# tiiuae/MLAdversarialObjectDetection

Hardware: AMD Instinct MI355X
Metric: patch-opt images/sec (EffDet-D0 512px fwd+bwd) (higher is better)
Workload: dtype f32; 1 GPU; C2: EfficientDet-D0 patch attack 512x512, 16 images/GPU, bn=local; global_batch=16, image_size=512, placement=injected, parallelism=dp1

## Files before the change

mladversarialobjectdetection_amd/csrc/api.cpp:

```cpp
#include "ctx.hpp"

namespace {

std::string json_escape(const std::string& s) {
  std::string o;
  for (char c : s) {
    if (c == '"' || c == '\\') o.push_back('\\');
    o.push_back(c);
  }
  return o;
}

std::vector<float> make_anchors(const ModelConfig& mc) {
  std::vector<int> fs{mc.image_size};
  int f = mc.image_size;
  for (int l = 1; l <= mc.max_level; ++l) {
    f = (f - 1) / 2 + 1;
    fs.push_back(f);
  }
  std::vector<float> out;
  for (int level = mc.min_level; level <= mc.max_level; ++level) {
    const double stride = (double)fs[0] / (double)fs[level];
    struct C { double base_x, base_y, ax, ay; };
    std::vector<C> cs;
// ... 589 lines not shown
  run_nms(ctx, E, 1, E.nms2_boxes, E.nms2_scores, E.nms2_count, s);
  launch_count_ge(E.nms2_scores, E.nms2_count, B, PHX_MAX_OUT, 0.5f, metrics + PHX_M_ASR_NUM, s);
  launch_tv(params, PHX_PATCH_SIZE, E.tvs, metrics, add_tv != 0, s);
  if (out_boxes) PHX_HIP(hipMemcpyAsync(out_boxes, E.nms2_boxes, (size_t)B * PHX_MAX_OUT * 16, hipMemcpyDeviceToDevice, s));
  if (out_scores) PHX_HIP(hipMemcpyAsync(out_scores, E.nms2_scores, (size_t)B * PHX_MAX_OUT * 4, hipMemcpyDeviceToDevice, s));
  if (out_count) PHX_HIP(hipMemcpyAsync(out_count, E.nms2_count, (size_t)B * 4, hipMemcpyDeviceToDevice, s));
  return PHX_OK;
  PHX_CATCH(ctx)
}

int phx_profile(phx_ctx* ctx, int enable) {
  if (!ctx) return PHX_EINVAL;
  ctx->prof.on = enable != 0;
  ctx->prof.recs.clear();
  ctx->prof.used = 0;
  return PHX_OK;
}

int phx_profile_report(phx_ctx* ctx, char* buf, size_t cap, size_t* needed) {
  if (!ctx) return PHX_EINVAL;
  PHX_TRY(ctx)
  if (buf && cap && !ctx->prof.report.empty()) {
    const std::string out = std::move(ctx->prof.report);
    ctx->prof.report.clear();
    if (needed) *needed = out.size() + 1;
    const size_t c = std::min(cap - 1, out.size());
    memcpy(buf, out.data(), c);
    buf[c] = 0;
    return PHX_OK;
  }
// ... 179 lines not shown
```

mladversarialobjectdetection_amd/csrc/ctx.hpp:

```cpp
#pragma once
#include <hip/hip_runtime.h>

#include <algorithm>
#include <array>
#include <cmath>
#include <cstdlib>
#include <cstring>
#include <exception>
#include <map>
#include <memory>
#include <sstream>
#include <string>
#include <functional>
#include <vector>

#include "common.hpp"
#include "env.hpp"
#include "exec_plan.hpp"
#include "kernels.hpp"
#include "model.hpp"
#include "phx.h"
#include "post.hpp"
#include "unet.hpp"

// ... 284 lines not shown
  size_t idx;
  hipStream_t s;
  std::string dbg;
  ExtTiming ext;
  Scope(phx_ctx* ctx, const char* kind, double flops, double bytes, hipStream_t st, const std::string& tag = "")
      : p(ctx->prof.on ? &ctx->prof : nullptr), s(st) {
    if (debug_sync()) {
      dbg = std::string(kind) + tag;
      PHX_HIP(hipStreamSynchronize(s));
    }
    if (!p) return;
    const double peak = (ctx->bf16 && std::string(kind) == "gemm") ? 2500.0 : 157.3;
    Prof::Rec r{std::string(kind) + (prof_detail() ? tag : std::string()), p->ev(), p->ev(), flops, bytes, peak};
    PHX_HIP(hipEventRecord(r.a, s));
    p->recs.push_back(r);
    idx = p->recs.size() - 1;
    if (std::string(kind) == "gemm") {
      ext = ExtTiming{r.a, r.b, false};
      ext_timing() = &ext;
    }
  }
  ~Scope() noexcept(false) {
    if (p) {
      if (ext_timing() == &ext) ext_timing() = nullptr;
      if (!ext.used) (void)hipEventRecord(p->recs[idx].b, s);
    }
    if (!dbg.empty() && std::uncaught_exceptions() == 0) {
      const hipError_t e = hipStreamSynchronize(s);
      if (e != hipSuccess) throw HipError(std::string("device error after ") + dbg + ": " + hipGetErrorString(e));
    }
// ... 34 lines not shown
```

mladversarialobjectdetection_amd/csrc/exec.cpp:

```cpp
#include "ctx.hpp"

constexpr size_t kMaxExecs = 4;

namespace {

void alloc_exec(Exec& E, int A) {
  const Program& P = E.prog;
  const int B = E.B;
  E.act = E.alloc<float>(E.abf ? (P.act_floats + 1) / 2 : P.act_floats);
  E.grad = E.alloc<float>(E.tag != 0 ? 1 : P.grad_floats);
  E.slot_a.assign(P.n_slots, nullptr);
  E.slot_b.assign(P.n_slots, nullptr);
  E.slot_c.assign(P.n_slots, nullptr);
  E.slot_d.assign(P.n_slots, nullptr);
  E.slot_e.assign(P.n_slots, nullptr);
  for (const Op& op : P.ops) {
    const Tensor& ti = P.tensors[op.in[0]];
    if (op.t == OP_BN) {
      E.slot_a[op.slot] = E.alloc<float>(ti.c);
      E.slot_b[op.slot] = E.alloc<float>(ti.c);
      E.slot_c[op.slot] = E.alloc<float>(ti.c);
      E.slot_d[op.slot] = E.alloc<float>(ti.c);
      E.slot_e[op.slot] = E.alloc<float>(ti.c);
      PHX_HIP(hipMemset(E.slot_d[op.slot], 0, ti.c * sizeof(float)));
// ... 957 lines not shown

}

phx::ExtTiming*& phx::ext_timing() {
  static ExtTiming* t = nullptr;
  return t;
}

phx::ProfScope phx::prof_begin(phx_ctx* ctx, const char* kind, double flops, double bytes, hipStream_t s) {
  ProfScope r{nullptr, 0, s};
  if (!ctx || !ctx->prof.on) return r;
  Prof* p = &ctx->prof;
  Prof::Rec rec{kind, p->ev(), p->ev(), flops, bytes, 157.3};
  PHX_HIP(hipEventRecord(rec.a, s));
  p->recs.push_back(rec);
  r.p = p;
  r.idx = p->recs.size() - 1;
  return r;
}

void phx::prof_end(const ProfScope& r) {
  if (r.p) PHX_HIP(hipEventRecord(static_cast<Prof*>(r.p)->recs[r.idx].b, r.s));
}
```

mladversarialobjectdetection_amd/csrc/kernels.hpp:

```cpp
#pragma once
#include <hip/hip_runtime.h>
#include <hip/hip_ext.h>

#include <cstddef>
#include <cstdint>

#include "common.hpp"

namespace phx {

struct ExtTiming {
  hipEvent_t a = nullptr, b = nullptr;
  bool used = false;
};
ExtTiming*& ext_timing();
#define PHX_TLAUNCH(K, G, BL, SHM, S, ...)                                                              \
  do {                                                                                                 \
    if (::phx::ExtTiming* t_ = ::phx::ext_timing()) {                                                  \
      hipExtLaunchKernelGGL(K, G, BL, SHM, S, t_->used ? nullptr : t_->a, t_->b, 0, __VA_ARGS__);      \
      t_->used = true;                                                                                 \
    } else {                                                                                           \
      hipLaunchKernelGGL(K, G, BL, SHM, S, __VA_ARGS__);                                               \
    }                                                                                                  \
  } while (0)
// ... 101 lines not shown
};
bool sep_bwd_supported(int C, int N, bool bf16);
void launch_sep_bwd(const SepBwdMember* m, int n, int B, int C, int N, const float* wd, const float* wp,
                    hipStream_t s, int* nps);
void launch_dw_fwd_fused(const FuseView& fv, const float* w, float* y, int B, int H, int W, int C, int Ho,
                         int Wo, int k, int stride, int pt, int pl, hipStream_t s);
void launch_dw_bwd_group(const DwSeg* segs, int n, int B, int C, const float* w, int k, int stride,
                         hipStream_t s, int* nps);
struct DwTileInfo {
  int lcg, rpt, otw, oth, nrg, rin, cin, tiles_x, ntiles, ncg;
  int small;
  long wgs;
};
DwTileInfo dw_tile_info(int H, int W, int C, int Ho, int Wo, int pt, int pl, int k, int stride, bool bwd);
DwTileInfo dw_fused_tile_info(int B, int H, int W, int C, int Ho, int Wo, int pt, int pl);
struct SepTileInfo {
  int tw, th, tiles_x, ntiles;
};
SepTileInfo sep_tile_info(int H, int W);
struct StemPlanInfo {
  int blocks, last_valid, tiles_x, tiles_y, last_qx, last_qy;
};
StemPlanInfo stem_plan_info(int B, int H, int W);
struct Conv3PlanInfo {
  int G, xr, sweeps;
  long tiles, tper;
  int xcd_tiles[8], xcd_wgs[8];
};
Conv3PlanInfo conv3_small_plan_info(long M);

// ... 161 lines not shown
```

mladversarialobjectdetection_amd/csrc/kernels_dw.hip:

```cpp
#include <algorithm>
#include <cstdlib>
#include <stdexcept>
#include <type_traits>

#include "env.hpp"
#include "dw_stage.hpp"
#include "kernels.hpp"

namespace phx {

struct DwGeom {
  int H, W, C;
  int Ho, Wo;
  int pt, pl;
  int lcg;
  int otw, oth;
  int nrg;
  int rin, cin;
  int tiles_x, ntiles, ncg;
  int per;
};

template <class XV>
struct DwFwdSegT {
  XV x;
  float* y;
  DwGeom g;
  StatSink sink;
};
using DwFwdSeg = DwFwdSegT<InX>;
template <int NS, class XV = InX>
struct DwFwdGroup {
  DwFwdSegT<XV> s[NS];
  const float* w;
};
// ... 75 lines not shown
}

template <class Src, int U = 4>
__device__ __forceinline__ void dw_stage(float4* tile, const Src& src, int b, int sh, int sw, int C,
                                         int r0, int c0, int chan, const DwGeom& g) {
  if constexpr (Src::kActT) {
    const int act = src.act();
    if (act == 1) dw_stage_t<1, Src, U>(tile, src, b, sh, sw, C, r0, c0, chan, g);
    else if (act == 2) dw_stage_t<2, Src, U>(tile, src, b, sh, sw, C, r0, c0, chan, g);
    else dw_stage_t<0, Src, U>(tile, src, b, sh, sw, C, r0, c0, chan, g);
  } else {
    dw_stage_t<0, Src, U>(tile, src, b, sh, sw, C, r0, c0, chan, g);
  }
}

__device__ __forceinline__ float4 dw_xor_sum(float4 v, int lcg) {
  for (int o = 1 << lcg; o < 64; o <<= 1) {
    v.x += __shfl_xor(v.x, o);
    v.y += __shfl_xor(v.y, o);
    v.z += __shfl_xor(v.z, o);
    v.w += __shfl_xor(v.w, o);
  }
  return v;
}

template <int RPT>
__device__ __forceinline__ void dw_stats(const float4 (&acc)[RPT], unsigned vmask, int lcg, int c,
                                         long p, const StatSink& sink) {
  __shared__ float4 wm_[4][8], w2_[4][8];
  __shared__ float wn_[4][8];
// ... 27 lines not shown
#pragma unroll
    for (int w = 0; w < 4; ++w) {
      const float4 a = wm_[w][cg], b = w2_[w][cg];
      const float nn = wn_[w][cg];
      chan_merge(tn[0], tm[0], t2[0], nn, a.x, b.x);
      chan_merge(tn[1], tm[1], t2[1], nn, a.y, b.y);
      chan_merge(tn[2], tm[2], t2[2], nn, a.z, b.z);
      chan_merge(tn[3], tm[3], t2[3], nn, a.w, b.w);
    }
#pragma unroll
    for (int j = 0; j < 4; ++j) sink_put(sink, p, c + j, tn[j], tm[j], t2[j]);
    if (threadIdx.x == 0) sink_cnt(sink, p, tn[0]);
  }
}

template <int K, int S, int RPT, bool STATS, int NS, class XV, int SU = 4, bool BF = false>
__global__ __launch_bounds__(256) void k_dw_fwd(DwFwdGroup<NS, XV> grp) {
  using Stage = std::conditional_t<std::is_same<XV, InX>::value, StageInX<BF>, StageFuse<BF>>;
  const DwFwdSegT<XV> sg = pick_seg(grp.s, NS == 1 ? 0 : (int)blockIdx.y);
  const XV& xv = sg.x;
  const DwGeom& g = sg.g;
  const StatSink& sink = sg.sink;
  const float* __restrict__ w = grp.w;
  float* __restrict__ y = sg.y;
  extern __shared__ float4 tile[];
  const int b = blockIdx.z;
  int tl, cgi;
  if (!dw_block_map(blockIdx.x, g.per, g.ncg, g.ntiles * g.ncg, &tl, &cgi)) return;
  const int CG = 1 << g.lcg;
  const int ty = tl / g.tiles_x, tx = tl - ty * g.tiles_x;
  const int oy0 = ty * g.oth, ox0 = tx * g.otw;
  const int cg = threadIdx.x & (CG - 1), q = threadIdx.x >> g.lcg;
  const int col = q % g.otw, rg = q / g.otw;
  const int c = (cgi * CG + cg) * 4;

  Stage src;
  src.init(xv, c);
  float4* wt = tile + g.rin * g.cin * CG;
  Taps<K> wr;
  wr.stage(wt, w, g.C, cgi, g.lcg);
  dw_stage<Stage, SU>(tile, src, b, g.H, g.W, g.C, oy0 * S - g.pt, ox0 * S - g.pl, c, g);
  __syncthreads();

  const int ox = ox0 + col;
  const int row0 = rg * RPT;
  const bool active = rg < g.nrg && ox < g.Wo && oy0 + row0 < g.Ho;
  if (!STATS && !active) return;
  float4 acc[RPT];
#pragma unroll
  for (int r = 0; r < RPT; ++r) acc[r] = make_float4(0.f, 0.f, 0.f, 0.f);
  if (active) {
    wr.init(wt, w, g.C, c, cg, g.lcg);
    constexpr int NR = (RPT - 1) * S + K;
    const float4* base = tile + ((row0 * S) * g.cin + col * S) * CG + cg;
#pragma unroll
    for (int ir = 0; ir < NR; ++ir) {
#pragma unroll
      for (int j = 0; j < K; ++j) {
        const float4 v = base[(ir * g.cin + j) * CG];
#pragma unroll
        for (int r = 0; r < RPT; ++r) {
          const int i = ir - r * S;
          if (i >= 0 && i < K) fma4(acc[r], v, wr(i * K + j));
        }
      }
      if constexpr (K > 3) __builtin_amdgcn_sched_barrier(0);
    }
  }
  unsigned vmask = 0;
#pragma unroll
  for (int r = 0; r < RPT; ++r) {
    const int oy = oy0 + row0 + r;
    if (active && oy < g.Ho) {
      vmask |= 1u << r;
      ast4<BF>(y, (((long)b * g.Ho + oy) * g.Wo + ox) * g.C + c, acc[r]);
    }
    if constexpr (BF && STATS)
      acc[r] = make_float4(round_bf16(acc[r].x), round_bf16(acc[r].y), round_bf16(acc[r].z), round_bf16(acc[r].w));
  }
  if constexpr (STATS) {
    dw_stats<RPT>(acc, vmask, g.lcg, c, (long)b * g.ntiles + tl, sink);
  }
}

__device__ __forceinline__ void dw_gsums(float4 s1, float4 s2, int lcg, int c, long p, const GradSink& g) {
  __shared__ float4 a_[4][8], b_[4][8];
  const int CG = 1 << lcg, cg = threadIdx.x & (CG - 1);
  const int lane = threadIdx.x & 63, wave = threadIdx.x >> 6;
  s1 = dw_xor_sum(s1, lcg);
  s2 = dw_xor_sum(s2, lcg);
  if (lane < CG) {
    a_[wave][cg] = s1;
    b_[wave][cg] = s2;
  }
  __syncthreads();
  if (threadIdx.x < CG) {
    float4 t1 = a_[0][cg], t2 = b_[0][cg];
#pragma unroll
    for (int w = 1; w < 4; ++w) {
      const float4 u = a_[w][cg], v = b_[w][cg];
      t1.x += u.x; t1.y += u.y; t1.z += u.z; t1.w += u.w;
      t2.x += v.x; t2.y += v.y; t2.z += v.z; t2.w += v.w;
    }
    gsink_put(g, p, c + 0, t1.x, t2.x);
    gsink_put(g, p, c + 1, t1.y, t2.y);
    gsink_put(g, p, c + 2, t1.z, t2.z);
    gsink_put(g, p, c + 3, t1.w, t2.w);
  }
}

template <int K, int S, int RPT, bool GS, int NS, int SU = 4, bool YBF = false>
__global__ __launch_bounds__(256) void k_dw_bwd(DwBwdGroup<NS> grp) {
  const DwBwdSeg sg = pick_seg(grp.s, NS == 1 ? 0 : (int)blockIdx.y);
  const GradX& gv = sg.gv;
  const DwGeom& g = sg.g;
  const GradSink& gsk = sg.gs;
  const int acc_flag = sg.acc;
  const float* __restrict__ w = grp.w;
  float* __restrict__ dx = sg.dx;
  extern __shared__ float4 tile[];
  const int b = blockIdx.z;
  int tl, cgi;
  if (!dw_block_map(blockIdx.x, g.per, g.ncg, g.ntiles * g.ncg, &tl, &cgi)) return;
  const int CG = 1 << g.lcg;
  const int ty = tl / g.tiles_x, tx = tl - ty * g.tiles_x;
  const int iy0 = ty * g.oth, ix0 = tx * g.otw;
  const int cg = threadIdx.x & (CG - 1), q = threadIdx.x >> g.lcg;
  const int col = q % g.otw, rg = q / g.otw;
  const int c = (cgi * CG + cg) * 4;
  const int ay = iy0 + g.pt - (K - 1), ax = ix0 + g.pl - (K - 1);
  const int oy_lo = S == 1 ? ay : (ay >= 0 ? ay / S : -((-ay + S - 1) / S));
  const int ox_lo = S == 1 ? ax : (ax >= 0 ? ax / S : -((-ax + S - 1) / S));

  StageGradX<YBF> src;
  src.init(gv, c);
  float4* wt = tile + g.rin * g.cin * CG;
  Taps<K> wr;
  wr.stage(wt, w, g.C, cgi, g.lcg);
  dw_stage<StageGradX<YBF>, SU>(tile, src, b, g.Ho, g.Wo, g.C, oy_lo, ox_lo, c, g);
  __syncthreads();

  const int ix = ix0 + col;
  const int row0 = rg * RPT;
  const bool active = rg < g.nrg && ix < g.W && iy0 + row0 < g.H;
  if (!GS && !active) return;
  float4 acc[RPT];
#pragma unroll
  for (int r = 0; r < RPT; ++r) acc[r] = make_float4(0.f, 0.f, 0.f, 0.f);
  if (active) {
    wr.init(wt, w, g.C, c, cg, g.lcg);
    if constexpr (S == 1) {
      constexpr int NR = RPT + K - 1;
      const float4* base = tile + (row0 * g.cin + col) * CG + cg;
#pragma unroll
      for (int ir = 0; ir < NR; ++ir) {
#pragma unroll
        for (int jj = 0; jj < K; ++jj) {
          const float4 v = base[(ir * g.cin + jj) * CG];
#pragma unroll
          for (int r = 0; r < RPT; ++r) {
            const int ii = ir - r;
            if (ii >= 0 && ii < K) fma4(acc[r], v, wr((K - 1 - ii) * K + (K - 1 - jj)));
          }
        }
        if constexpr (K > 3) __builtin_amdgcn_sched_barrier(0);
      }
    } else {
      const int u0 = ix + g.pl;
#pragma unroll
      for (int r = 0; r < RPT; ++r) {
        const int t0 = iy0 + row0 + r + g.pt;
#pragma unroll
        for (int i = 0; i < K; ++i) {
          const int t = t0 - i;
          if (t & 1) continue;
          const int lr = (t >> 1) - oy_lo;
#pragma unroll
          for (int j = 0; j < K; ++j) {
            const int u = u0 - j;
            if (u & 1) continue;
            const int lc = (u >> 1) - ox_lo;
            fma4(acc[r], tile[(lr * g.cin + lc) * CG + cg], wr(i * K + j));
          }
        }
      }
    }
  }
  float4 s1 = make_float4(0.f, 0.f, 0.f, 0.f), s2 = s1;
  GSChan4 kk;
  if (GS && active) kk = gs_chan4(gsk, c);
  float4 old[RPT], yv[RPT];
  const int ixc = min(ix, g.W - 1);
#pragma unroll
  for (int r = 0; r < RPT; ++r) {
    const long e = (((long)b * g.H + min(iy0 + row0 + r, g.H - 1)) * g.W + ixc) * g.C + c;
    if (acc_flag) old[r] = *reinterpret_cast<const float4*>(dx + e);
    if constexpr (GS) yv[r] = ald4<YBF>(gsk.y, e);
  }
#pragma unroll
  for (int r = 0; r < RPT; ++r) {
    const int iy = iy0 + row0 + r;
    if (!active || iy >= g.H) continue;
    const long e = (((long)b * g.H + iy) * g.W + ix) * g.C + c;
    float4* o = reinterpret_cast<float4*>(dx + e);
    float4 a = acc[r];
    if (acc_flag) {
      a.x += old[r].x; a.y += old[r].y; a.z += old[r].z; a.w += old[r].w;
    }
    *o = a;
    if constexpr (GS) gs_acc4(gsk, kk, a, yv[r], s1, s2);
  }
  if constexpr (GS) {
    dw_gsums(s1, s2, g.lcg, c, (long)b * g.ntiles + tl, gsk);
  }
}

static int dw_rpt_fwd(int stride) { return stride == 1 ? 4 : 2; }

static int dw_lcg(int C, int k, int s, bool bwd) {
  static int env_cap = [] {
    const char* e = std::getenv("PHX_DW_MAXLCG");
    return e ? std::min(3, std::max(0, atoi(e))) : -1;
  }();
  const int cap = env_cap >= 0 ? env_cap : ((!bwd && s == 1) || (bwd && k == 5)) ? 2 : 3;
  const int c4 = C / 4;
  const int l = (c4 % 8 == 0) ? 3 : (c4 % 4 == 0) ? 2 : (c4 % 2 == 0) ? 1 : 0;
  return std::min(l, cap);
}
// ... 13 lines not shown
  if (!bwd) {
    g.rin = (g.oth - 1) * s + k;
    g.cin = (g.otw - 1) * s + k;
  } else {
    g.rin = (g.oth - 1 + k - 1) / s + 2;
    g.cin = (g.otw - 1 + k - 1) / s + 2;
    if (s == 1) {
      g.rin = g.oth + k - 1;
      g.cin = g.otw + k - 1;
    }
  }
  g.tiles_x = cdiv(ow, g.otw);
  g.ntiles = g.tiles_x * cdiv(oh, g.oth);
  g.ncg = C / (4 << g.lcg);
  g.per = cdiv((long)g.ntiles * g.ncg, 8);
  return g;
}

static size_t dw_lds(const DwGeom& g, int k) {
  const bool lds_taps = PHX_DW_LDS_TAPS == 2 || (PHX_DW_LDS_TAPS == 1 && k > 3);
  return ((size_t)g.rin * g.cin + (lds_taps ? k * k : 0)) * (1 << g.lcg) * sizeof(float4);
}

static bool xv_bf(const InX& x) { return x.bf != 0; }
static bool xv_bf(const FuseView& f) { return f.x[0].bf != 0; }

template <int K, int S, int RPT, int NS, class XV, int SU, bool BF>
static void dw_fwd_launch(dim3 grid, size_t lds, const DwFwdGroup<NS, XV>& grp, bool stats, hipStream_t s) {
  if (stats) hipLaunchKernelGGL((k_dw_fwd<K, S, RPT, true, NS, XV, SU, BF>), grid, dim3(256), lds, s, grp);
  else hipLaunchKernelGGL((k_dw_fwd<K, S, RPT, false, NS, XV, SU, BF>), grid, dim3(256), lds, s, grp);
}

template <int K, int S, int RPT, int NS, class XV>
static void dw_fwd_go(const DwFwdGroup<NS, XV>& grp, int n, int B, bool stats, hipStream_t s) {
  const bool bf = xv_bf(grp.s[0].x);
  int gx = 1;
  size_t lds = 0;
  for (int i = 0; i < n; ++i) {
    gx = std::max(gx, 8 * grp.s[i].g.per);
    lds = std::max(lds, dw_lds(grp.s[i].g, K));
  }
  dim3 grid(gx, n, B);
  if constexpr (S == 2 || std::is_same<XV, InX>::value) {
// ... 20 lines not shown

int dw_stat_partials(int B, int H, int W, int C, int Ho, int Wo, int k, int stride, int pt, int pl) {
  const int rpt = dw_rpt_fwd(stride);
  DwGeom g = dw_plan(H, W, C, Ho, Wo, pt, pl, k, stride, rpt, false);
  return B * g.ntiles;
}

int launch_dw_fwd(InX x, const float* w, float* y, int B, int H, int W, int C, int Ho, int Wo,
                  int k, int stride, int pt, int pl, hipStream_t s, StatSink sink) {
  if (C % 4) throw std::runtime_error("dw: C % 4 != 0");
  const int rpt = dw_rpt_fwd(stride);
  DwFwdGroup<1> grp{};
  grp.w = w;
  grp.s[0] = DwFwdSeg{x, y, dw_plan(H, W, C, Ho, Wo, pt, pl, k, stride, rpt, false), sink};
  grp.s[0].sink.P = B * grp.s[0].g.ntiles;
  dw_fwd_dispatch(grp, 1, B, sink.part != nullptr, k, stride, s);
  return B * grp.s[0].g.ntiles;
}

static bool dw_fused_small(int B, const DwGeom& g) {
  static const long small_below = env_long("PHX_DW_FUSE_SMALL", 512L);
  return (long)B * g.ntiles * g.ncg < small_below;
}

void launch_dw_fwd_fused(const FuseView& fv, const float* w, float* y, int B, int H, int W, int C, int Ho,
                         int Wo, int k, int stride, int pt, int pl, hipStream_t s) {
  if (C % 4) throw std::runtime_error("dw: C % 4 != 0");
  if (k != 3 || stride != 1) throw std::invalid_argument("dw fused: 3x3 stride 1 only");
  DwFwdGroup<1, FuseView> grp{};
  grp.w = w;
// ... 26 lines not shown
    nps[i] = grp.s[i].sink.P;
  }
  dw_fwd_dispatch(grp, n, B, stats, k, stride, s);
}

template <int K, int S, int NS>
static void dw_bwd_go(const DwBwdGroup<NS>& grp, int n, int B, bool gsums, hipStream_t s) {
  int gx = 1;
  size_t lds = 0;
  for (int i = 0; i < n; ++i) {
    gx = std::max(gx, 8 * grp.s[i].g.per);
    lds = std::max(lds, dw_lds(grp.s[i].g, K));
  }
  dim3 grid(gx, n, B);
  const bool ybf = (grp.s[0].gv.y && grp.s[0].gv.ybf) || (gsums && grp.s[0].gs.ybf);
  if (ybf) {
    if (gsums)
      hipLaunchKernelGGL((k_dw_bwd<K, S, 4, true, NS, 4, true>), grid, dim3(256), lds, s, grp);
    else
      hipLaunchKernelGGL((k_dw_bwd<K, S, 4, false, NS, 4, true>), grid, dim3(256), lds, s, grp);
    return;
  }
  if (gsums)
    hipLaunchKernelGGL((k_dw_bwd<K, S, 4, true, NS>), grid, dim3(256), lds, s, grp);
  else
    hipLaunchKernelGGL((k_dw_bwd<K, S, 4, false, NS>), grid, dim3(256), lds, s, grp);
}

template <int NS>
static void dw_bwd_dispatch(const DwBwdGroup<NS>& grp, int n, int B, bool gsums, int k, int stride,
// ... 8 lines not shown
  PHX_LAUNCH_CHECK();
}

int dw_bwd_partials(int B, int H, int W, int C, int Ho, int Wo, int k, int stride, int pt, int pl) {
  DwGeom g = dw_plan(H, W, C, Ho, Wo, pt, pl, k, stride, 4, true);
  return B * g.ntiles;
}

int launch_dw_bwd(GradX dy, const float* w, float* dx, int B, int H, int W, int C, int Ho,
                  int Wo, int k, int stride, int pt, int pl, bool acc, hipStream_t s, GradSink gs) {
  if (C % 4) throw std::runtime_error("dw: C % 4 != 0");
  DwBwdGroup<1> grp{};
  grp.w = w;
  grp.s[0] = DwBwdSeg{dy, dx, dw_plan(H, W, C, Ho, Wo, pt, pl, k, stride, 4, true), acc ? 1 : 0, gs};
  grp.s[0].gs.P = B * grp.s[0].g.ntiles;
  dw_bwd_dispatch(grp, 1, B, gs.part != nullptr, k, stride, s);
  return B * grp.s[0].g.ntiles;
}

void launch_dw_bwd_group(const DwSeg* segs, int n, int B, int C, const float* w, int k, int stride,
                         hipStream_t s, int* nps) {
  if (C % 4) throw std::runtime_error("dw: C % 4 != 0");
  if (n < 1 || n > kMaxSeg) throw std::runtime_error("dw group: bad member count");
  DwBwdGroup<kMaxSeg> grp{};
  grp.w = w;
  const bool gsums = segs[0].gs.part != nullptr;
  for (int i = 0; i < n; ++i) {
    const DwSeg& d = segs[i];
    if ((d.gs.part != nullptr) != gsums) throw std::runtime_error("dw group: members differ in sinks");
    grp.s[i] = DwBwdSeg{d.gv, d.out, dw_plan(d.H, d.W, C, d.Ho, d.Wo, d.pt, d.pl, k, stride, 4, true),
// ... 1 lines not shown
    grp.s[i].gs.P = B * grp.s[i].g.ntiles;
    nps[i] = grp.s[i].gs.P;
  }
  dw_bwd_dispatch(grp, n, B, gsums, k, stride, s);
}

static DwTileInfo dw_info_of(const DwGeom& g, int rpt) {
  return DwTileInfo{g.lcg, rpt, g.otw, g.oth, g.nrg, g.rin, g.cin, g.tiles_x, g.ntiles, g.ncg, 0, 0};
}

DwTileInfo dw_tile_info(int H, int W, int C, int Ho, int Wo, int pt, int pl, int k, int stride, bool bwd) {
  const int rpt = bwd ? 4 : dw_rpt_fwd(stride);
  return dw_info_of(dw_plan(H, W, C, Ho, Wo, pt, pl, k, stride, rpt, bwd), rpt);
}

DwTileInfo dw_fused_tile_info(int B, int H, int W, int C, int Ho, int Wo, int pt, int pl) {
  const DwGeom g = dw_plan(H, W, C, Ho, Wo, pt, pl, 3, 1, 4, false);
  const bool small = dw_fused_small(B, g);
  DwTileInfo t = small ? dw_info_of(dw_plan(H, W, C, Ho, Wo, pt, pl, 3, 1, 1, false, 0), 1) : dw_info_of(g, 4);
  t.small = small ? 1 : 0;
  t.wgs = (long)B * g.ntiles * g.ncg;
  return t;
}

}
```

mladversarialobjectdetection_amd/csrc/kernels_eot.hip:

```cpp
#include "common.hpp"
#include "env.hpp"
#include "post.hpp"

#pragma clang fp contract(off)

#include "span.hpp"

namespace phx {

__device__ __forceinline__ u32x4 rng(uint64_t seed, uint32_t c0, uint32_t c1, uint32_t c2,
                                     int64_t step, uint32_t stream) {
  return philox4x32_10(u32x4{c0, c1, c2, (uint32_t)((uint64_t)step << 8) | stream},
                       (uint32_t)seed, (uint32_t)(seed >> 32));
}
__device__ __forceinline__ float runif(uint32_t v, float lo, float hi) {
  return u01(v) * (hi - lo) + lo;
}
__device__ __forceinline__ float rnorm(uint32_t a, uint32_t b, float mean, float sd) {
  float u1 = u01_open0(a), u2 = u01(b);
  float z = sqrtf(-2.0f * logf(u1)) * cosf(6.28318530717958647692f * u2);
  return z * sd + mean;
}

struct EotLists {
// ... 534 lines not shown
  }
  return lo;
}

constexpr int kBoxGrid = 2048;

constexpr int kResizeGrid = 1280;

__global__ __launch_bounds__(256) void k_eot_resize(EotDims d, const float* __restrict__ matched,
                                                    const BoxPlace* __restrict__ place,
                                                    const SpanEntry* __restrict__ spans,
                                                    uint64_t seed, int64_t step, int gimg0,
                                                    float* __restrict__ rstore, float amp) {
  extern __shared__ float V[];
  const ListView L = lists_of(d, place);
  const int xb = blockIdx.x & 7;
  int* const bx = reinterpret_cast<int*>(V + kResizeRT * d.P * 3);
  if (threadIdx.x == 0) bx[0] = 0;
  for (int b0 = 0; b0 < d.B; b0 += 256) {
    __shared__ int sx[256];
    const int bb = b0 + (int)threadIdx.x;
    sx[threadIdx.x] = bb < d.B ? L.bcnt[xb * d.B + bb] : 0;
    __syncthreads();
    for (int off = 1; off < 256; off <<= 1) {
      const int a = threadIdx.x >= (unsigned)off ? sx[threadIdx.x - off] : 0;
      __syncthreads();
      sx[threadIdx.x] += a;
      __syncthreads();
    }
    if (bb < d.B) bx[bb + 1] = bx[b0] + sx[threadIdx.x];
    __syncthreads();
  }
  const int* bv = L.bvpre + xb * d.B * d.maxb;
  const int total = bx[d.B];
  for (int item = blockIdx.x >> 3; item < total; item += gridDim.x >> 3) {
    int b = 0;
    {
      int lo = 0, hi = d.B - 1;
      while (lo < hi) {
        const int mid = (lo + hi + 1) >> 1;
        if (bx[mid] <= item) lo = mid; else hi = mid - 1;
      }
      b = lo;
    }
    const int local = item - bx[b];
    const int v = L.img_first[b] + find_box(bv + L.img_first[b], L.img_n[b], local);
    const int sl = L.vlist[v];
    const BoxPlace P = place[sl];
    const int k = sl % d.maxb;
    const int nt = (P.ps + kResizeRT - 1) / kResizeRT;
    const int i0 = (xb * nt / 8 + (local - bv[v])) * kResizeRT;
    const int ni = min(kResizeRT, P.ps - i0);
    const SpanEntry* sp = spans + (long)sl * d.span_stride;
    const float scale = (float)P.ps / (float)d.P;
    const float inv_scale = (float)(1.0 / (double)scale);
    const float one_over_k = 1.0f / fmaxf(inv_scale, 1.0f);
    const int xlo = sp[0].start, nx = sp[P.ps - 1].end - xlo;
    const float* m = matched + (long)b * d.P * d.P * 3;
    const int h2 = (nx + 1) >> 1;
    for (int e2 = threadIdx.x; e2 < ni * h2; e2 += blockDim.x) {
      const int ii = e2 / h2, xa = e2 - ii * h2, xb = xa + h2;
      const bool okb = xb < nx;
      const SpanEntry si = sp[i0 + ii];
      const float* ca = m + (long)(xlo + xa) * 3;
      const float* cb = m + (long)(xlo + (okb ? xb : xa)) * 3;
      float a0 = 0.f, a1 = 0.f, a2 = 0.f, b0 = 0.f, b1 = 0.f, b2 = 0.f;
// ... 895 lines not shown
```

Measured before the change: 1459 images/s.

## Add row-marching depthwise conv kernels that reuse a ring-buffered LDS tile

Adds a MARCH mode to the depthwise forward and backward kernels. Each block walks several vertically adjacent tiles and keeps the input rows in LDS as a ring buffer, prefetching only the new rows into registers while computing the current tile. This cuts redundant halo loads and per-block staging overhead, at the cost of fewer blocks, more registers and extra LDS for parked loader parameters. By default it is enabled only for forward launches with stride other than 1 that have enough work items; the backward path is opt-in through an environment variable. Also includes small profiling report-clearing fixes and a variable rename in the EOT resize kernel.

```diff
diff --git a/mladversarialobjectdetection_amd/csrc/api.cpp b/mladversarialobjectdetection_amd/csrc/api.cpp
--- a/mladversarialobjectdetection_amd/csrc/api.cpp
+++ b/mladversarialobjectdetection_amd/csrc/api.cpp
@@ -627,6 +627,7 @@
   ctx->prof.on = enable != 0;
   ctx->prof.recs.clear();
   ctx->prof.used = 0;
+  ctx->prof.report.clear();
   return PHX_OK;
 }
 
diff --git a/mladversarialobjectdetection_amd/csrc/ctx.hpp b/mladversarialobjectdetection_amd/csrc/ctx.hpp
--- a/mladversarialobjectdetection_amd/csrc/ctx.hpp
+++ b/mladversarialobjectdetection_amd/csrc/ctx.hpp
@@ -322,6 +322,7 @@
     Prof::Rec r{std::string(kind) + (prof_detail() ? tag : std::string()), p->ev(), p->ev(), flops, bytes, peak};
     PHX_HIP(hipEventRecord(r.a, s));
     p->recs.push_back(r);
+    p->report.clear();
     idx = p->recs.size() - 1;
     if (std::string(kind) == "gemm") {
       ext = ExtTiming{r.a, r.b, false};
diff --git a/mladversarialobjectdetection_amd/csrc/exec.cpp b/mladversarialobjectdetection_amd/csrc/exec.cpp
--- a/mladversarialobjectdetection_amd/csrc/exec.cpp
+++ b/mladversarialobjectdetection_amd/csrc/exec.cpp
@@ -995,6 +995,7 @@
   Prof::Rec rec{kind, p->ev(), p->ev(), flops, bytes, 157.3};
   PHX_HIP(hipEventRecord(rec.a, s));
   p->recs.push_back(rec);
+  p->report.clear();
   r.p = p;
   r.idx = p->recs.size() - 1;
   return r;
diff --git a/mladversarialobjectdetection_amd/csrc/kernels.hpp b/mladversarialobjectdetection_amd/csrc/kernels.hpp
--- a/mladversarialobjectdetection_amd/csrc/kernels.hpp
+++ b/mladversarialobjectdetection_amd/csrc/kernels.hpp
@@ -139,6 +139,7 @@
 };
 DwTileInfo dw_tile_info(int H, int W, int C, int Ho, int Wo, int pt, int pl, int k, int stride, bool bwd);
 DwTileInfo dw_fused_tile_info(int B, int H, int W, int C, int Ho, int Wo, int pt, int pl);
+int dw_march_tiles(int B, int H, int W, int C, int Ho, int Wo, int pt, int pl, int k, int stride, bool bwd);
 struct SepTileInfo {
   int tw, th, tiles_x, ntiles;
 };
diff --git a/mladversarialobjectdetection_amd/csrc/kernels_dw.hip b/mladversarialobjectdetection_amd/csrc/kernels_dw.hip
--- a/mladversarialobjectdetection_amd/csrc/kernels_dw.hip
+++ b/mladversarialobjectdetection_amd/csrc/kernels_dw.hip
@@ -19,6 +19,8 @@
   int rin, cin;
   int tiles_x, ntiles, ncg;
   int per;
+  int nt;
+  int mper;
 };
 
 template <class XV>
@@ -124,6 +126,83 @@
   }
 }
 
+constexpr int dw_march_pf(int S, bool bwd) { return bwd ? (S == 1 ? 5 : 3) : (S == 1 ? 5 : 9); }
+constexpr int kDwMarchParkF4 = 6;
+template <class Src>
+__device__ __forceinline__ void dw_march_park(float4* kl, const Src& src, int cg) {
+  using KT = decltype(src.k);
+  static_assert(sizeof(KT) <= kDwMarchParkF4 * sizeof(float4), "parked parameters");
+  if ((int)threadIdx.x == cg) reinterpret_cast<KT*>(kl)[cg] = src.k;
+}
+template <class Src>
+__device__ __forceinline__ void dw_march_unpark(const float4* kl, Src& src, int cg) {
+  using KT = decltype(src.k);
+  src.k = reinterpret_cast<const KT*>(kl)[cg];
+}
+
+template <int PF>
+__device__ __forceinline__ void dw_march_init(int (&pk)[PF], const DwGeom& g) {
+  const int pstep = 256 >> g.lcg;
+  const int p = threadIdx.x >> g.lcg;
+#pragma unroll
+  for (int u = 0; u < PF; ++u) {
+    const int pp = p + u * pstep;
+    const int prow = pp / g.cin;
+    pk[u] = (prow << 16) | (pp - prow * g.cin);
+  }
+}
+
+template <class Src, int PF>
+__device__ __forceinline__ void dw_march_load(typename Src::Raw (&v)[PF], const int (&pk)[PF], const Src& src,
+                                              int b, int sh, int sw, int C, int r0, int c0, int chan, int nrow) {
+#pragma unroll
+  for (int u = 0; u < PF; ++u) {
+    const int prow = pk[u] >> 16, pcol = pk[u] & 0xffff;
+    const int iyc = min(max(r0 + prow, 0), sh - 1), ixc = min(max(c0 + pcol, 0), sw - 1);
+    if (prow < nrow) v[u] = src.load((((long)b * sh + iyc) * sw + ixc) * C + chan);
+    else v[u] = src.zero();
+  }
+}
+
+template <int ACT, class Src, int PF>
+__device__ __forceinline__ void dw_march_put_t(float4* tile, const typename Src::Raw (&v)[PF], const int (&pk)[PF],
+                                               const Src& src, int sh, int sw, int r0, int c0, int nrow, int head,
+                                               const DwGeom& g) {
+  const int ecg = threadIdx.x & ((1 << g.lcg) - 1);
+#pragma unroll
+  for (int u = 0; u < PF; ++u) {
+    const int prow = pk[u] >> 16, pcol = pk[u] & 0xffff;
+    const int iy = r0 + prow, ix = c0 + pcol;
+    const bool ok = iy >= 0 && iy < sh && ix >= 0 && ix < sw;
+    int slot = head + prow;
+    slot -= slot >= g.rin ? g.rin : 0;
+    if (prow < nrow)
+      tile[((slot * g.cin + pcol) << g.lcg) + ecg] = ok ? src.template finish_t<ACT>(v[u]) : make_float4(0.f, 0.f, 0.f, 0.f);
+  }
+}
+
+template <class Src, int PF>
+__device__ __forceinline__ void dw_march_put(float4* tile, const typename Src::Raw (&v)[PF], const int (&pk)[PF],
+                                             const Src& src, int sh, int sw, int r0, int c0, int nrow, int head,
+                                             const DwGeom& g) {
+  const int act = src.act();
+  if (act == 1) dw_march_put_t<1, Src, PF>(tile, v, pk, src, sh, sw, r0, c0, nrow, head, g);
+  else if (act == 2) dw_march_put_t<2, Src, PF>(tile, v, pk, src, sh, sw, r0, c0, nrow, head, g);
+  else dw_march_put_t<0, Src, PF>(tile, v, pk, src, sh, sw, r0, c0, nrow, head, g);
+}
+
+__device__ __forceinline__ bool dw_march_map(const DwGeom& g, int* ty, int* tx, int* nt, int* cgi) {
+  const int tiles_y = g.ntiles / g.tiles_x;
+  const int nseg = (tiles_y + g.nt - 1) / g.nt;
+  int item;
+  if (!dw_block_map(blockIdx.x, g.mper, g.ncg, g.tiles_x * nseg * g.ncg, &item, cgi)) return false;
+  const int sgm = item / g.tiles_x;
+  *tx = item - sgm * g.tiles_x;
+  *ty = sgm * g.nt;
+  *nt = min(g.nt, tiles_y - *ty);
+  return true;
+}
+
 __device__ __forceinline__ float4 dw_xor_sum(float4 v, int lcg) {
   for (int o = 1 << lcg; o < 64; o <<= 1) {
     v.x += __shfl_xor(v.x, o);
@@ -181,8 +260,9 @@
   }
 }
 
-template <int K, int S, int RPT, bool STATS, int NS, class XV, int SU = 4, bool BF = false>
+template <int K, int S, int RPT, bool STATS, int NS, class XV, int SU = 4, bool BF = false, bool MARCH = false>
 __global__ __launch_bounds__(256) void k_dw_fwd(DwFwdGroup<NS, XV> grp) {
+  static_assert(!MARCH || (NS == 1 && std::is_same<XV, InX>::value), "marching: ungrouped InX launches only");
   using Stage = std::conditional_t<std::is_same<XV, InX>::value, StageInX<BF>, StageFuse<BF>>;
   const DwFwdSegT<XV> sg = pick_seg(grp.s, NS == 1 ? 0 : (int)blockIdx.y);
   const XV& xv = sg.x;
@@ -192,11 +272,18 @@
   float* __restrict__ y = sg.y;
   extern __shared__ float4 tile[];
   const int b = blockIdx.z;
-  int tl, cgi;
-  if (!dw_block_map(blockIdx.x, g.per, g.ncg, g.ntiles * g.ncg, &tl, &cgi)) return;
+  int tl, cgi, ty, tx, nt = 1;
+  if constexpr (MARCH) {
+    if (!dw_march_map(g, &ty, &tx, &nt, &cgi)) return;
+    tl = ty * g.tiles_x + tx;
+  } else {
+    if (!dw_block_map(blockIdx.x, g.per, g.ncg, g.ntiles * g.ncg, &tl, &cgi)) return;
+    ty = tl / g.tiles_x;
+    tx = tl - ty * g.tiles_x;
+  }
   const int CG = 1 << g.lcg;
-  const int ty = tl / g.tiles_x, tx = tl - ty * g.tiles_x;
-  const int oy0 = ty * g.oth, ox0 = tx * g.otw;
+  int oy0 = ty * g.oth;
+  const int ox0 = tx * g.otw;
   const int cg = threadIdx.x & (CG - 1), q = threadIdx.x >> g.lcg;
   const int col = q % g.otw, rg = q / g.otw;
   const int c = (cgi * CG + cg) * 4;
@@ -206,47 +293,86 @@
   float4* wt = tile + g.rin * g.cin * CG;
   Taps<K> wr;
   wr.stage(wt, w, g.C, cgi, g.lcg);
+  [[maybe_unused]] float4* kl = wt + K * K * CG;
+  if constexpr (MARCH) dw_march_park(kl, src, cg);
   dw_stage<Stage, SU>(tile, src, b, g.H, g.W, g.C, oy0 * S - g.pt, ox0 * S - g.pl, c, g);
   __syncthreads();
 
   const int ox = ox0 + col;
   const int row0 = rg * RPT;
-  const bool active = rg < g.nrg && ox < g.Wo && oy0 + row0 < g.Ho;
-  if (!STATS && !active) return;
-  float4 acc[RPT];
-#pragma unroll
-  for (int r = 0; r < RPT; ++r) acc[r] = make_float4(0.f, 0.f, 0.f, 0.f);
-  if (active) {
-    wr.init(wt, w, g.C, c, cg, g.lcg);
-    constexpr int NR = (RPT - 1) * S + K;
-    const float4* base = tile + ((row0 * S) * g.cin + col * S) * CG + cg;
-#pragma unroll
-    for (int ir = 0; ir < NR; ++ir) {
-#pragma unroll
-      for (int j = 0; j < K; ++j) {
-        const float4 v = base[(ir * g.cin + j) * CG];
-#pragma unroll
-        for (int r = 0; r < RPT; ++r) {
-          const int i = ir - r * S;
-          if (i >= 0 && i < K) fma4(acc[r], v, wr(i * K + j));
+  constexpr int PF = MARCH ? dw_march_pf(S, false) : 1;
+  [[maybe_unused]] typename Stage::Raw pv[PF];
+  [[maybe_unused]] int pk[PF];
+  [[maybe_unused]] int head = 0;
+  [[maybe_unused]] const int adv = g.oth * S;
+  if constexpr (MARCH) dw_march_init<PF>(pk, g);
+  for (int t = 0;; ++t) {
+    const bool more = MARCH && t + 1 < nt;
+    [[maybe_unused]] const int nr0 = oy0 * S - g.pt + g.rin;
+    if constexpr (MARCH) {
+      if (more) dw_march_load<Stage, PF>(pv, pk, src, b, g.H, g.W, g.C, nr0, ox0 * S - g.pl, c, adv);
+    }
+    const bool active = rg < g.nrg && ox < g.Wo && oy0 + row0 < g.Ho;
+    if constexpr (!MARCH) {
+      if (!STATS && !active) return;
+    }
+    float4 acc[RPT];
+#pragma unroll
+    for (int r = 0; r < RPT; ++r) acc[r] = make_float4(0.f, 0.f, 0.f, 0.f);
+    if (active) {
+      wr.init(wt, w, g.C, c, cg, g.lcg);
+      constexpr int NR = (RPT - 1) * S + K;
+      const float4* base = tile + ((row0 * S) * g.cin + col * S) * CG + cg;
+      [[maybe_unused]] const float4* colb = tile + (col * S) * CG + cg;
+      [[maybe_unused]] int rs = head + row0 * S;
+      if constexpr (MARCH) rs -= rs >= g.rin ? g.rin : 0;
+#pragma unroll
+      for (int ir = 0; ir < NR; ++ir) {
+        const float4* rowp;
+        if constexpr (MARCH) {
+          int rr = rs + ir;
+          rr -= rr >= g.rin ? g.rin : 0;
+          rowp = colb + rr * g.cin * CG;
+        } else {
+          rowp = base + ir * g.cin * CG;
         }
+#pragma unroll
+        for (int j = 0; j < K; ++j) {
+          const float4 v = rowp[j * CG];
+#pragma unroll
+          for (int r = 0; r < RPT; ++r) {
+            const int i = ir - r * S;
+            if (i >= 0 && i < K) fma4(acc[r], v, wr(i * K + j));
+          }
+        }
+        if constexpr (K > 3) __builtin_amdgcn_sched_barrier(0);
       }
-      if constexpr (K > 3) __builtin_amdgcn_sched_barrier(0);
-    }
-  }
-  unsigned vmask = 0;
-#pragma unroll
-  for (int r = 0; r < RPT; ++r) {
-    const int oy = oy0 + row0 + r;
-    if (active && oy < g.Ho) {
-      vmask |= 1u << r;
-      ast4<BF>(y, (((long)b * g.Ho + oy) * g.Wo + ox) * g.C + c, acc[r]);
-    }
-    if constexpr (BF && STATS)
-      acc[r] = make_float4(round_bf16(acc[r].x), round_bf16(acc[r].y), round_bf16(acc[r].z), round_bf16(acc[r].w));
-  }
-  if constexpr (STATS) {
-    dw_stats<RPT>(acc, vmask, g.lcg, c, (long)b * g.ntiles + tl, sink);
+    }
+    unsigned vmask = 0;
+#pragma unroll
+    for (int r = 0; r < RPT; ++r) {
+      const int oy = oy0 + row0 + r;
+      if (active && oy < g.Ho) {
+        vmask |= 1u << r;
+        ast4<BF>(y, (((long)b * g.Ho + oy) * g.Wo + ox) * g.C + c, acc[r]);
+      }
+      if constexpr (BF && STATS)
+        acc[r] = make_float4(round_bf16(acc[r].x), round_bf16(acc[r].y), round_bf16(acc[r].z), round_bf16(acc[r].w));
+    }
+    if constexpr (STATS) {
+      dw_stats<RPT>(acc, vmask, g.lcg, c, (long)b * g.ntiles + tl, sink);
+    }
+    if (!more) break;
+    if constexpr (MARCH) {
+      if constexpr (!STATS) __syncthreads();
+      dw_march_unpark(kl, src, cg);
+      dw_march_put<Stage, PF>(tile, pv, pk, src, g.H, g.W, nr0, ox0 * S - g.pl, adv, head, g);
+      __syncthreads();
+      head += adv;
+      head -= head >= g.rin ? g.rin : 0;
+      oy0 += g.oth;
+      tl += g.tiles_x;
+    }
   }
 }
 
@@ -276,8 +402,10 @@
   }
 }
 
-template <int K, int S, int RPT, bool GS, int NS, int SU = 4, bool YBF = false>
+template <int K, int S, int RPT, bool GS, int NS, int SU = 4, bool YBF = false, bool MARCH = false>
 __global__ __launch_bounds__(256) void k_dw_bwd(DwBwdGroup<NS> grp) {
+  static_assert(!MARCH || NS == 1, "marching: ungrouped launches only");
+  static_assert(RPT % S == 0, "a tile's rows advance the dy window by whole rows");
   const DwBwdSeg sg = pick_seg(grp.s, NS == 1 ? 0 : (int)blockIdx.y);
   const GradX& gv = sg.gv;
   const DwGeom& g = sg.g;
@@ -287,16 +415,23 @@
   float* __restrict__ dx = sg.dx;
   extern __shared__ float4 tile[];
   const int b = blockIdx.z;
-  int tl, cgi;
-  if (!dw_block_map(blockIdx.x, g.per, g.ncg, g.ntiles * g.ncg, &tl, &cgi)) return;
+  int tl, cgi, ty, tx, nt = 1;
+  if constexpr (MARCH) {
+    if (!dw_march_map(g, &ty, &tx, &nt, &cgi)) return;
+    tl = ty * g.tiles_x + tx;
+  } else {
+    if (!dw_block_map(blockIdx.x, g.per, g.ncg, g.ntiles * g.ncg, &tl, &cgi)) return;
+    ty = tl / g.tiles_x;
+    tx = tl - ty * g.tiles_x;
+  }
   const int CG = 1 << g.lcg;
-  const int ty = tl / g.tiles_x, tx = tl - ty * g.tiles_x;
-  const int iy0 = ty * g.oth, ix0 = tx * g.otw;
+  int iy0 = ty * g.oth;
+  const int ix0 = tx * g.otw;
   const int cg = threadIdx.x & (CG - 1), q = threadIdx.x >> g.lcg;
   const int col = q % g.otw, rg = q / g.otw;
   const int c = (cgi * CG + cg) * 4;
   const int ay = iy0 + g.pt - (K - 1), ax = ix0 + g.pl - (K - 1);
-  const int oy_lo = S == 1 ? ay : (ay >= 0 ? ay / S : -((-ay + S - 1) / S));
+  int oy_lo = S == 1 ? ay : (ay >= 0 ? ay / S : -((-ay + S - 1) / S));
   const int ox_lo = S == 1 ? ax : (ax >= 0 ? ax / S : -((-ax + S - 1) / S));
 
   StageGradX<YBF> src;
@@ -304,81 +439,125 @@
   float4* wt = tile + g.rin * g.cin * CG;
   Taps<K> wr;
   wr.stage(wt, w, g.C, cgi, g.lcg);
+  [[maybe_unused]] float4* kl = wt + K * K * CG;
+  if constexpr (MARCH) dw_march_park(kl, src, cg);
   dw_stage<StageGradX<YBF>, SU>(tile, src, b, g.Ho, g.Wo, g.C, oy_lo, ox_lo, c, g);
   __syncthreads();
 
   const int ix = ix0 + col;
   const int row0 = rg * RPT;
-  const bool active = rg < g.nrg && ix < g.W && iy0 + row0 < g.H;
-  if (!GS && !active) return;
-  float4 acc[RPT];
-#pragma unroll
-  for (int r = 0; r < RPT; ++r) acc[r] = make_float4(0.f, 0.f, 0.f, 0.f);
-  if (active) {
-    wr.init(wt, w, g.C, c, cg, g.lcg);
-    if constexpr (S == 1) {
-      constexpr int NR = RPT + K - 1;
-      const float4* base = tile + (row0 * g.cin + col) * CG + cg;
-#pragma unroll
-      for (int ir = 0; ir < NR; ++ir) {
-#pragma unroll
-        for (int jj = 0; jj < K; ++jj) {
-          const float4 v = base[(ir * g.cin + jj) * CG];
-#pragma unroll
-          for (int r = 0; r < RPT; ++r) {
-            const int ii = ir - r;
-            if (ii >= 0 && ii < K) fma4(acc[r], v, wr((K - 1 - ii) * K + (K - 1 - jj)));
+  constexpr int PF = MARCH ? dw_march_pf(S, true) : 1;
+  [[maybe_unused]] typename StageGradX<YBF>::Raw pv[PF];
+  [[maybe_unused]] int pk[PF];
+  [[maybe_unused]] int head = 0;
+  [[maybe_unused]] const int adv = g.oth / S;
+  if constexpr (MARCH) dw_march_init<PF>(pk, g);
+  for (int t = 0;; ++t) {
+    const bool more = MARCH && t + 1 < nt;
+    [[maybe_unused]] const int nr0 = oy_lo + g.rin;
+    if constexpr (MARCH) {
+      if (more) dw_march_load<StageGradX<YBF>, PF>(pv, pk, src, b, g.Ho, g.Wo, g.C, nr0, ox_lo, c, adv);
+    }
+    const bool active = rg < g.nrg && ix < g.W && iy0 + row0 < g.H;
+    if constexpr (!MARCH) {
+      if (!GS && !active) return;
+    }
+    float4 acc[RPT];
+#pragma unroll
+    for (int r = 0; r < RPT; ++r) acc[r] = make_float4(0.f, 0.f, 0.f, 0.f);
+    if (active) {
+      wr.init(wt, w, g.C, c, cg, g.lcg);
+      if constexpr (S == 1) {
+        constexpr int NR = RPT + K - 1;
+        const float4* base = tile + (row0 * g.cin + col) * CG + cg;
+        [[maybe_unused]] const float4* colb = tile + col * CG + cg;
+        [[maybe_unused]] int rs = head + row0;
+        if constexpr (MARCH) rs -= rs >= g.rin ? g.rin : 0;
+#pragma unroll
+        for (int ir = 0; ir < NR; ++ir) {
+          const float4* rowp;
+          if constexpr (MARCH) {
+            int rr = rs + ir;
+            rr -= rr >= g.rin ? g.rin : 0;
+            rowp = colb + rr * g.cin * CG;
+          } else {
+            rowp = base + ir * g.cin * CG;
           }
+#pragma unroll
+          for (int jj = 0; jj < K; ++jj) {
+            const float4 v = rowp[jj * CG];
+#pragma unroll
+            for (int r = 0; r < RPT; ++r) {
+              const int ii = ir - r;
+              if (ii >= 0 && ii < K) fma4(acc[r], v, wr((K - 1 - ii) * K + (K - 1 - jj)));
+            }
+          }
+          if constexpr (K > 3) __builtin_amdgcn_sched_barrier(0);
         }
-        if constexpr (K > 3) __builtin_amdgcn_sched_barrier(0);
-      }
-    } else {
-      const int u0 = ix + g.pl;
-#pragma unroll
-      for (int r = 0; r < RPT; ++r) {
-        const int t0 = iy0 + row0 + r + g.pt;
-#pragma unroll
-        for (int i = 0; i < K; ++i) {
-          const int t = t0 - i;
-          if (t & 1) continue;
-          const int lr = (t >> 1) - oy_lo;
-#pragma unroll
-          for (int j = 0; j < K; ++j) {
-            const int u = u0 - j;
-            if (u & 1) continue;
-            const int lc = (u >> 1) - ox_lo;
-            fma4(acc[r], tile[(lr * g.cin + lc) * CG + cg], wr(i * K + j));
+      } else {
+        const int u0 = ix + g.pl;
+#pragma unroll
+        for (int r = 0; r < RPT; ++r) {
+          const int t0 = iy0 + row0 + r + g.pt;
+#pragma unroll
+          for (int i = 0; i < K; ++i) {
+            const int tt = t0 - i;
+            if (tt & 1) continue;
+            int lr = (tt >> 1) - oy_lo;
+            if constexpr (MARCH) {
+              lr += head;
+              lr -= lr >= g.rin ? g.rin : 0;
+            }
+#pragma unroll
+            for (int j = 0; j < K; ++j) {
+              const int u = u0 - j;
+              if (u & 1) continue;
+              const int lc = (u >> 1) - ox_lo;
+              fma4(acc[r], tile[(lr * g.cin + lc) * CG + cg], wr(i * K + j));
+            }
           }
         }
       }
     }
-  }
-  float4 s1 = make_float4(0.f, 0.f, 0.f, 0.f), s2 = s1;
-  GSChan4 kk;
-  if (GS && active) kk = gs_chan4(gsk, c);
-  float4 old[RPT], yv[RPT];
-  const int ixc = min(ix, g.W - 1);
-#pragma unroll
-  for (int r = 0; r < RPT; ++r) {
-    const long e = (((long)b * g.H + min(iy0 + row0 + r, g.H - 1)) * g.W + ixc) * g.C + c;
-    if (acc_flag) old[r] = *reinterpret_cast<const float4*>(dx + e);
-    if constexpr (GS) yv[r] = ald4<YBF>(gsk.y, e);
-  }
-#pragma unroll
-  for (int r = 0; r < RPT; ++r) {
-    const int iy = iy0 + row0 + r;
-    if (!active || iy >= g.H) continue;
-    const long e = (((long)b * g.H + iy) * g.W + ix) * g.C + c;
-    float4* o = reinterpret_cast<float4*>(dx + e);
-    float4 a = acc[r];
-    if (acc_flag) {
-      a.x += old[r].x; a.y += old[r].y; a.z += old[r].z; a.w += old[r].w;
-    }
-    *o = a;
-    if constexpr (GS) gs_acc4(gsk, kk, a, yv[r], s1, s2);
-  }
-  if constexpr (GS) {
-    dw_gsums(s1, s2, g.lcg, c, (long)b * g.ntiles + tl, gsk);
+    float4 s1 = make_float4(0.f, 0.f, 0.f, 0.f), s2 = s1;
+    GSChan4 kk;
+    if (GS && active) kk = gs_chan4(gsk, c);
+    float4 old[RPT], yv[RPT];
+    const int ixc = min(ix, g.W - 1);
+#pragma unroll
+    for (int r = 0; r < RPT; ++r) {
+      const long e = (((long)b * g.H + min(iy0 + row0 + r, g.H - 1)) * g.W + ixc) * g.C + c;
+      if (acc_flag) old[r] = *reinterpret_cast<const float4*>(dx + e);
+      if constexpr (GS) yv[r] = ald4<YBF>(gsk.y, e);
+    }
+#pragma unroll
+    for (int r = 0; r < RPT; ++r) {
+      const int iy = iy0 + row0 + r;
+      if (!active || iy >= g.H) continue;
+      const long e = (((long)b * g.H + iy) * g.W + ix) * g.C + c;
+      float4* o = reinterpret_cast<float4*>(dx + e);
+      float4 a = acc[r];
+      if (acc_flag) {
+        a.x += old[r].x; a.y += old[r].y; a.z += old[r].z; a.w += old[r].w;
+      }
+      *o = a;
+      if constexpr (GS) gs_acc4(gsk, kk, a, yv[r], s1, s2);
+    }
+    if constexpr (GS) {
+      dw_gsums(s1, s2, g.lcg, c, (long)b * g.ntiles + tl, gsk);
+    }
+    if (!more) break;
+    if constexpr (MARCH) {
+      if constexpr (!GS) __syncthreads();
+      dw_march_unpark(kl, src, cg);
+      dw_march_put<StageGradX<YBF>, PF>(tile, pv, pk, src, g.Ho, g.Wo, nr0, ox_lo, adv, head, g);
+      __syncthreads();
+      head += adv;
+      head -= head >= g.rin ? g.rin : 0;
+      oy_lo += adv;
+      iy0 += g.oth;
+      tl += g.tiles_x;
+    }
   }
 }
 
@@ -422,12 +601,40 @@
   g.ntiles = g.tiles_x * cdiv(oh, g.oth);
   g.ncg = C / (4 << g.lcg);
   g.per = cdiv((long)g.ntiles * g.ncg, 8);
+  g.nt = 1;
+  g.mper = g.per;
   return g;
+}
+
+constexpr long kDwMarchMinItems = 2048;
+
+static bool dw_march_fits(const DwGeom& g, int s, bool bwd) {
+  if (bwd && g.oth % s) return false;
+  const int adv = bwd ? g.oth / s : g.oth * s;
+  return adv <= g.rin && cdiv(adv * g.cin, 256 >> g.lcg) <= dw_march_pf(s, bwd);
+}
+
+static void dw_march_plan(DwGeom& g, int B, int s, bool bwd) {
+  const char* e = std::getenv("PHX_DW_MARCH");
+  const int tiles_y = g.ntiles / g.tiles_x;
+  int nt = 1;
+  if (e && e[0] == '0') return;
+  if (tiles_y < 2 || !dw_march_fits(g, s, bwd)) return;
+  if (e && e[0] == 'a') {
+    nt = tiles_y <= 4 ? 2 : 8;
+  } else {
+    if (bwd || s == 1) return;
+    for (int cand = 8; cand >= 2 && nt == 1; cand >>= 1)
+      if ((long)B * g.tiles_x * cdiv(tiles_y, cand) * g.ncg >= kDwMarchMinItems) nt = cand;
+  }
+  if (nt == 1) return;
+  g.nt = nt;
+  g.mper = cdiv((long)g.tiles_x * cdiv(tiles_y, nt) * g.ncg, 8);
 }
 
 static size_t dw_lds(const DwGeom& g, int k) {
   const bool lds_taps = PHX_DW_LDS_TAPS == 2 || (PHX_DW_LDS_TAPS == 1 && k > 3);
-  return ((size_t)g.rin * g.cin + (lds_taps ? k * k : 0)) * (1 << g.lcg) * sizeof(float4);
+  return ((size_t)g.rin * g.cin + (lds_taps ? k * k : 0) + (g.nt > 1 ? kDwMarchParkF4 : 0)) * (1 << g.lcg) * sizeof(float4);
 }
 
 static bool xv_bf(const InX& x) { return x.bf != 0; }
@@ -435,6 +642,14 @@
 
 template <int K, int S, int RPT, int NS, class XV, int SU, bool BF>
 static void dw_fwd_launch(dim3 grid, size_t lds, const DwFwdGroup<NS, XV>& grp, bool stats, hipStream_t s) {
+  if constexpr (NS == 1 && std::is_same<XV, InX>::value) {
+    if (grp.s[0].g.nt > 1) {
+      grid.x = 8 * grp.s[0].g.mper;
+      if (stats) hipLaunchKernelGGL((k_dw_fwd<K, S, RPT, true, NS, XV, SU, BF, true>), grid, dim3(256), lds, s, grp);
+      else hipLaunchKernelGGL((k_dw_fwd<K, S, RPT, false, NS, XV, SU, BF, true>), grid, dim3(256), lds, s, grp);
+      return;
+    }
+  }
   if (stats) hipLaunchKernelGGL((k_dw_fwd<K, S, RPT, true, NS, XV, SU, BF>), grid, dim3(256), lds, s, grp);
   else hipLaunchKernelGGL((k_dw_fwd<K, S, RPT, false, NS, XV, SU, BF>), grid, dim3(256), lds, s, grp);
 }
@@ -485,6 +700,7 @@
   grp.w = w;
   grp.s[0] = DwFwdSeg{x, y, dw_plan(H, W, C, Ho, Wo, pt, pl, k, stride, rpt, false), sink};
   grp.s[0].sink.P = B * grp.s[0].g.ntiles;
+  dw_march_plan(grp.s[0].g, B, stride, false);
   dw_fwd_dispatch(grp, 1, B, sink.part != nullptr, k, stride, s);
   return B * grp.s[0].g.ntiles;
 }
@@ -541,6 +757,20 @@
   }
   dim3 grid(gx, n, B);
   const bool ybf = (grp.s[0].gv.y && grp.s[0].gv.ybf) || (gsums && grp.s[0].gs.ybf);
+  if constexpr (NS == 1) {
+    if (grp.s[0].g.nt > 1) {
+      grid.x = 8 * grp.s[0].g.mper;
+      if (ybf && gsums)
+        hipLaunchKernelGGL((k_dw_bwd<K, S, 4, true, NS, 4, true, true>), grid, dim3(256), lds, s, grp);
+      else if (ybf)
+        hipLaunchKernelGGL((k_dw_bwd<K, S, 4, false, NS, 4, true, true>), grid, dim3(256), lds, s, grp);
+      else if (gsums)
+        hipLaunchKernelGGL((k_dw_bwd<K, S, 4, true, NS, 4, false, true>), grid, dim3(256), lds, s, grp);
+      else
+        hipLaunchKernelGGL((k_dw_bwd<K, S, 4, false, NS, 4, false, true>), grid, dim3(256), lds, s, grp);
+      return;
+    }
+  }
   if (ybf) {
     if (gsums)
       hipLaunchKernelGGL((k_dw_bwd<K, S, 4, true, NS, 4, true>), grid, dim3(256), lds, s, grp);
@@ -579,6 +809,7 @@
   grp.w = w;
   grp.s[0] = DwBwdSeg{dy, dx, dw_plan(H, W, C, Ho, Wo, pt, pl, k, stride, 4, true), acc ? 1 : 0, gs};
   grp.s[0].gs.P = B * grp.s[0].g.ntiles;
+  dw_march_plan(grp.s[0].g, B, stride, true);
   dw_bwd_dispatch(grp, 1, B, gs.part != nullptr, k, stride, s);
   return B * grp.s[0].g.ntiles;
 }
@@ -610,6 +841,12 @@
   return dw_info_of(dw_plan(H, W, C, Ho, Wo, pt, pl, k, stride, rpt, bwd), rpt);
 }
 
+int dw_march_tiles(int B, int H, int W, int C, int Ho, int Wo, int pt, int pl, int k, int stride, bool bwd) {
+  DwGeom g = dw_plan(H, W, C, Ho, Wo, pt, pl, k, stride, bwd ? 4 : dw_rpt_fwd(stride), bwd);
+  dw_march_plan(g, B, stride, bwd);
+  return g.nt;
+}
+
 DwTileInfo dw_fused_tile_info(int B, int H, int W, int C, int Ho, int Wo, int pt, int pl) {
   const DwGeom g = dw_plan(H, W, C, Ho, Wo, pt, pl, 3, 1, 4, false);
   const bool small = dw_fused_small(B, g);
diff --git a/mladversarialobjectdetection_amd/csrc/kernels_eot.hip b/mladversarialobjectdetection_amd/csrc/kernels_eot.hip
--- a/mladversarialobjectdetection_amd/csrc/kernels_eot.hip
+++ b/mladversarialobjectdetection_amd/csrc/kernels_eot.hip
@@ -572,13 +572,13 @@
                                                     float* __restrict__ rstore, float amp) {
   extern __shared__ float V[];
   const ListView L = lists_of(d, place);
-  const int xb = blockIdx.x & 7;
+  const int band = blockIdx.x & 7;
   int* const bx = reinterpret_cast<int*>(V + kResizeRT * d.P * 3);
   if (threadIdx.x == 0) bx[0] = 0;
   for (int b0 = 0; b0 < d.B; b0 += 256) {
     __shared__ int sx[256];
     const int bb = b0 + (int)threadIdx.x;
-    sx[threadIdx.x] = bb < d.B ? L.bcnt[xb * d.B + bb] : 0;
+    sx[threadIdx.x] = bb < d.B ? L.bcnt[band * d.B + bb] : 0;
     __syncthreads();
     for (int off = 1; off < 256; off <<= 1) {
       const int a = threadIdx.x >= (unsigned)off ? sx[threadIdx.x - off] : 0;
@@ -589,7 +589,7 @@
     if (bb < d.B) bx[bb + 1] = bx[b0] + sx[threadIdx.x];
     __syncthreads();
   }
-  const int* bv = L.bvpre + xb * d.B * d.maxb;
+  const int* bv = L.bvpre + band * d.B * d.maxb;
   const int total = bx[d.B];
   for (int item = blockIdx.x >> 3; item < total; item += gridDim.x >> 3) {
     int b = 0;
@@ -607,7 +607,7 @@
     const BoxPlace P = place[sl];
     const int k = sl % d.maxb;
     const int nt = (P.ps + kResizeRT - 1) / kResizeRT;
-    const int i0 = (xb * nt / 8 + (local - bv[v])) * kResizeRT;
+    const int i0 = (band * nt / 8 + (local - bv[v])) * kResizeRT;
     const int ni = min(kResizeRT, P.ps - i0);
     const SpanEntry* sp = spans + (long)sl * d.span_stride;
     const float scale = (float)P.ps / (float)d.P;
```

New measurement: 1453 images/s. No clear change (-0.4%).
